# sp-uhh/disentangled-vae

Hardware: AMD Instinct MI355X
Metric: spectrogram frames/sec (train step), M2 VAE 513-bin (higher is better)
Workload: dtype bf16x3; 1 GPU; M2 VAE train step (fwd+ELBO+bwd+Adam), x_dim 513, y_dim 513, z 16, h [128,128], 8192 frames/step/GPU, 16 kHz / 1024-pt STFT power frames; parallelism=dp1, min_hbm_bytes_per_frame=4168

## Files before the change

### disentangled-vae_amd/csrc/rows_common.hpp

```cpp
#pragma once
#include "fused_tiles.hpp"
#include "apply_types.hpp"

namespace dvae {
namespace fused {

__device__ __forceinline__ void philox_normal4(unsigned long long seed, unsigned long long frame, unsigned long long step, unsigned draw,
                                               float (&out)[4]) {
    unsigned c0 = (unsigned)frame, c1 = (unsigned)(frame >> 32), c2 = (unsigned)step, c3 = ((unsigned)(step >> 32) << 8) | draw;
    unsigned k0 = (unsigned)seed, k1 = (unsigned)(seed >> 32);
#pragma unroll
    for (int r = 0; r < 10; ++r) {
        const unsigned h0 = __umulhi(0xD2511F53u, c0), l0 = 0xD2511F53u * c0;
        const unsigned h1 = __umulhi(0xCD9E8D57u, c2), l1 = 0xCD9E8D57u * c2;
        c0 = h1 ^ c1 ^ k0; c1 = l1; c2 = h0 ^ c3 ^ k1; c3 = l0;
        k0 += 0x9E3779B9u; k1 += 0xBB67AE85u;
    }
    const float u0 = ((float)(c0 >> 8) + 0.5f) * (1.f / 16777216.f), u1 = ((float)(c1 >> 8) + 0.5f) * (1.f / 16777216.f);
    const float u2 = ((float)(c2 >> 8) + 0.5f) * (1.f / 16777216.f), u3 = ((float)(c3 >> 8) + 0.5f) * (1.f / 16777216.f);
    const float ra = sqrtf(-2.f * __logf(u0)), rb = sqrtf(-2.f * __logf(u2));
    float sa, ca, sb, cb;
    __sincosf(6.283185307179586f * u1, &sa, &ca);
    __sincosf(6.283185307179586f * u3, &sb, &cb);
    out[0] = ra * ca; out[1] = ra * sa; out[2] = rb * cb; out[3] = rb * sb;
// ... 128 lines not shown
                if (fbase + l31 >= col_limit) f[j] = P::cvt(0.f);
            }
            stash_store16(dbase, (l31 * E + gq * 32 * E) * (int)sizeof(T), f);
        }
    }
}

template <typename P, bool F16 = false, typename RowOf>
__device__ __forceinline__ void load_rows_to_lds(const float* __restrict__ src, int ld, int ncols, int pcols, int64_t b0, int64_t B,
                                                 typename P::T* U, int ldu, int tid, RowOf rowof, float* xf = nullptr,
                                                 float* log2sum = nullptr, float eps = 0.f) {
    const int total = TB * pcols;
    for (int idx = tid; idx < total; idx += 256) {
        const int row = idx / pcols, col = idx - row * pcols;
        float v = 0.f;
        if (col < ncols && b0 + row < B) {
            v = src[rowof(row) * ld + col];
            if (log2sum && col < XD - 1) *log2sum += __builtin_amdgcn_logf(v + eps);
        }
        if constexpr (F16 && P::NP == 2) {
            const float vs = v * X16::XS;
            const typename P::T vh = X16::hi<typename P::T>(vs);
            U[row * ldu + col] = vh;
            U[Pl<P>::lds + row * ldu + col] = X16::hi<typename P::T>(vs - X16::val(vh));
        } else {
            const typename P::T vh = P::cvt(v);
            U[row * ldu + col] = vh;
            if constexpr (P::NP == 2) U[Pl<P>::lds + row * ldu + col] = P::cvt(v - (float)vh);
        }
        if (xf && col < ncols) xf[row * ncols + col] = v;
    }
}

constexpr int NQ513 = 17;
struct __attribute__((packed, aligned(4))) F4U { f32x4 v; };
#ifndef R2_IN_NT
#define R2_IN_NT 0
#endif
typedef f32x4 f32x4_a4 __attribute__((aligned(4)));
__device__ __forceinline__ f32x4 ld_in4(const float* p) {
#if R2_IN_NT >= 1
    return __builtin_nontemporal_load(reinterpret_cast<const f32x4_a4*>(p));
#else
    return reinterpret_cast<const F4U*>(p)->v;
#endif
}
__device__ __forceinline__ f32x4 ld_in4_again(const float* p) {
#if R2_IN_NT >= 2
    return __builtin_nontemporal_load(reinterpret_cast<const f32x4_a4*>(p));
#else
    return reinterpret_cast<const F4U*>(p)->v;
#endif
}
template <int I0, int I1, typename RowOf>
__device__ __forceinline__ void tile513_issue_part(const float* __restrict__ base, RowOf rowof, f32x4 (&v)[NQ513], int tid) {
#pragma unroll
    for (int i = I0; i < I1; ++i) {
        const int c = tid + 256 * i;
        v[i] = ld_in4(base + rowof(c >> 7) * XD + 4 * (c & 127));
    }
}
template <typename RowOf>
__device__ __forceinline__ void tile513_issue_last(const float* __restrict__ base, RowOf rowof, f32x4 (&v)[NQ513], int tid) {
    v[16][0] = base[rowof(tid & 31) * XD + XD - 1];
}
template <typename RowOf>
__device__ __forceinline__ void tile513_issue(const float* __restrict__ base, RowOf rowof, f32x4 (&v)[NQ513], int tid) {
    tile513_issue_part<0, 16>(base, rowof, v, tid);
    tile513_issue_last(base, rowof, v, tid);
    __builtin_amdgcn_sched_barrier(0);
}
template <typename P, int I0, int I1, bool F16 = false>
__device__ __forceinline__ void tile513_commit_part(const f32x4 (&v)[NQ513], typename P::T* U, int ldu, int tid, float* xf, unsigned long long& lo_bits) {
    typedef typename P::Pack4 Pack4;
#pragma unroll
    for (int i = I0; i < I1; ++i) {
        const int c = tid + 256 * i;
        const int row = c >> 7, col = 4 * (c & 127);
        if (xf) {
            float* d = xf + row * XD + col;
            d[0] = v[i][0]; d[1] = v[i][1]; d[2] = v[i][2]; d[3] = v[i][3];
        }
        if constexpr (F16 && P::NP == 2) {
            Pack4 pk, pl;
#pragma unroll
            for (int j = 0; j < 4; ++j) {
                const float vs = v[i][j] * X16::XS;
                pk[j] = X16::hi<typename P::T>(vs);
                pl[j] = X16::hi<typename P::T>(vs - X16::val(pk[j]));
            }
            *reinterpret_cast<Pack4*>(U + row * ldu + col) = pk;
            *reinterpret_cast<Pack4*>(U + Pl<P>::lds + row * ldu + col) = pl;
            continue;
        }
        Pack4 pk;
        pk[0] = P::cvt(v[i][0]); pk[1] = P::cvt(v[i][1]); pk[2] = P::cvt(v[i][2]); pk[3] = P::cvt(v[i][3]);
        *reinterpret_cast<Pack4*>(U + row * ldu + col) = pk;
        if constexpr (P::NP == 2) {
            Pack4 pl;
            pl[0] = P::cvt(v[i][0] - (float)pk[0]); pl[1] = P::cvt(v[i][1] - (float)pk[1]);
            pl[2] = P::cvt(v[i][2] - (float)pk[2]); pl[3] = P::cvt(v[i][3] - (float)pk[3]);
            *reinterpret_cast<Pack4*>(U + Pl<P>::lds + row * ldu + col) = pl;
            lo_bits |= __builtin_bit_cast(unsigned long long, pl) & 0x7fff7fff7fff7fffull;
        }
    }
}
template <typename P, int PCOLS, bool F16 = false>
__device__ __forceinline__ void tile513_commit_last(const f32x4 (&v)[NQ513], typename P::T* U, int ldu, int tid, float* xf, unsigned long long& lo_bits) {
    constexpr int PADC = PCOLS - XD;
    if (tid < TB) {
        if (xf) xf[tid * XD + XD - 1] = v[16][0];
// ... 107 lines not shown
```

### disentangled-vae_amd/csrc/rows_helper.inc

```
        const int hw = wave_u - ROWS_CHAIN_WAVES, ht = tid - 64 * ROWS_CHAIN_WAVES;
        constexpr bool XFH = P::XF16 && NP == 2;
        constexpr int NBT = Ld<T>::nbias;
        constexpr int NB = (NBT + 255) / 256;
        float bvv[NB];
        auto load_bias = [&]() __attribute__((always_inline)) {
#pragma unroll
            for (int q = 0; q < NB; ++q) {
                int i = ht + 256 * q;
                i = i < NBT ? i : NBT - 1;
                const float* src;
                int k;
                if (i < OB2) { src = g.b1; k = i; }
                else if (i < OBMV) { src = g.b2; k = i - OB2; }
                else if (i < OBMV + ZD) { src = g.bmu; k = i - OBMV; }
                else if (i < OB3) { src = g.blv; k = i - OBMV - ZD; }
                else if (i < OB4) { src = g.b3; k = i - OB3; }
                else if (i < OB5) { src = g.b4; k = i - OB4; }
                else if (i < OB5 + NO) { src = g.b5; k = i - OB5; k = k < XD ? k : XD - 1; }
                else { src = g.w5last; k = i - OB5 - NO; }
                if constexpr (DEFER) bvv[q] = __hip_atomic_load(src + k, __ATOMIC_RELAXED, __HIP_MEMORY_SCOPE_AGENT);
                else bvv[q] = src[k];
            }
        };
        auto store_bias = [&]() __attribute__((always_inline)) {
// ... 23 lines not shown
            hws.pl = g.wpl_bytes;
            auto mo = [&](const void* Wp) { return (unsigned)((const char*)Wp - (const char*)g.wcopy); };
            constexpr unsigned FBB = HS::FBB;
            const unsigned tw = (unsigned)hw * FBB;
            hws.sb[H_W1X] = mo(g.W1s) + tw + (unsigned)SCc::NX1 * 4u * FBB;
            hws.sb[H_W3Y] = mo(g.W3s) + tw + (unsigned)(ZD / KS) * 4u * FBB;
            hws.sb[H_W3Z] = mo(g.W3s) + tw;
            hws.sb[H_PAD] = mo(g.W1s);
            if constexpr (INFO) { hws.sb[H_C1] = mo(g.Wc1s) + tw;  hws.sb[H_C2] = mo(g.Wc2s) + tw;  hws.sb[H_C2T] = mo(g.Wc2t) + tw; }
            else { hws.sb[H_C1] = hws.sb[H_C2] = hws.sb[H_C2T] = 0; }
            if constexpr (INFO) hws.fill();
        }
        const T* const Urh = U + l31 * LDU + h * E;
        const T* const Zbrh = Zb + l31 * LDZ + h * E;
        float lsum2 = 0.f;
        f32x4 xv[NQ513], yv[NQ513];
        bool x_in_regs = false;
        bool y_in_regs = false;
        const bool st1 = MODE != 1 && !(g.ablate & 1), st2 = MODE != 1 && !(g.ablate & 2) && (g.stash_inputs & 2), st2x = MODE != 1 && !(g.ablate & 2) && (g.stash_inputs & 1);
        for (int it = 0; it < ntl; ++it) {
            const int tile = tile0 + it * (int)gridDim.x;
            const int64_t b0 = (int64_t)tile * TB;
            const bool full = (b0 + TB) <= g.B;
            const int64_t* const rsrc = rowsrc + (it & 1) * TB;
            auto rowof = [&](int r) -> int64_t {
                if (gather) return rsrc[r];
                const int64_t br = b0 + r;
                return br < g.B ? br : g.B - 1;
            };
            int tl = ht;
            asm volatile("" : "+v"(tl));
            const bool yfast = Y513 && g.fasty && full;
            bool y_early = it > 0 && y_in_regs;
            if (it == 0) {
                if (gather) { fill_rows(tile, 0); wg_barrier(); }
                if (g.fastx && full) {
                    tile513_issue(g.x, rowof, xv, tl);
                    if constexpr (!DEFER) store_bias();
#if R2_EARLY_Y
                    if (YP > 0 && Y513 && g.fasty) {
                        unsigned long long lb = 0ull;
                        static_for<0, 4>([&](auto qc) {
                            constexpr int Q = decltype(qc)::value;
                            tile513_issue_part<4 * Q, 4 * Q + 4>(g.y, rowof, yv, tl);
                            __builtin_amdgcn_sched_barrier(0);
                            tile513_commit_part<P, 4 * Q, 4 * Q + 4, XFH>(xv, U, LDU, tl, nullptr, lb);
                            __builtin_amdgcn_sched_barrier(0);
                        });
                        tile513_issue_last(g.y, rowof, yv, tl);
                        __builtin_amdgcn_sched_barrier(0);
                        tile513_commit_last<P, ROWS_XP, XFH>(xv, U, LDU, tl, nullptr, lb);
                        y_early = true;
                    } else
#endif
                    {
                        tile513_commit<P, ROWS_XP, XFH>(xv, U, LDU, tl);
#pragma unroll
                        for (int i = 0; i < NQ513; ++i) yv[i] = f32x4{0.f, 0.f, 0.f, 0.f};
                    }
                } else {
#pragma unroll
                    for (int i = 0; i < NQ513; ++i) { xv[i] = f32x4{0.f, 0.f, 0.f, 0.f}; yv[i] = f32x4{0.f, 0.f, 0.f, 0.f}; }
                    if constexpr (!DEFER) store_bias();
                    load_rows_to_lds<P, XFH>(g.x, g.ldx, XD, ROWS_XP, b0, g.B, U, LDU, tl, rowof, nullptr, OFFL ? &lsum2 : nullptr, g.elbo_eps);
                }
                if constexpr (INFO) {
                    for (int i = ht; i < 6 * HD + 2; i += 256) {
                        const int q = i / HD, k = i - q * HD;
                        float v;
                        if (q == 0) v = g.bc1[k]; else if (q == 1) v = g.bc2[k]; else if (q == 2) v = g.wc3[k];
                        else if (q == 3) v = g.ba1[k]; else if (q == 4) v = g.ba2[k]; else if (q == 5) v = g.wa3[k];
                        else v = k == 0 ? g.bc3[0] : g.ba3[0];
                        Binfo[i] = v;
                    }
                }
                if (ht == 0) flags[0] = 0;
                if constexpr (DEFER) {
                    wg_barrier();
                    load_bias();
                    store_bias();
                }
                wg_barrier();
                if constexpr (OFFL) { if (g.fastx && full) lsum2 += tile513_log2sum(xv, g.elbo_eps, tl); }
            }
            if constexpr (HS::n(H_W1X) > 0) {
                f32x16 hacc;
                zero_acc<P>(hacc);
                hws.fill();
                gemm_seg<P, HS, DH, H_W1X, HWS, XFH>(hacc, hws, Urh + SCc::NX1 * 2 * E);
#pragma unroll
                for (int r = 0; r < 16; ++r) keep[r * 256 + ht] = XFH ? hacc[r] * X16::ACC : hacc[r];
            }
            float c1r[16], c2r[16], w3c[16];
            float bce_c = 0.f, ylab = 0.f;
            if constexpr (INFO) {
                ylab = g.y[rowof(l31) * g.ldy];
                if (it > 0) hws.fill();
                f32x16 cacc;
                zero_acc<P>(cacc);
                gemm_seg<P, HS, DH, H_C1, HWS, XFH>(cacc, hws, Urh);
                float bvc[16];
                bias16(Binfo + OBC1, 32 * hw, h, bvc);
#pragma unroll
                for (int r = 0; r < 16; ++r) c1r[r] = fmaxf((XFH ? cacc[r] * X16::ACC : cacc[r]) + bvc[r], 0.f);
            }
            f32x16 accy;
            int yplanes = NP;
            int ydirty = 0;
            if constexpr (NP == 2 && YP > 0) { if (g.ylo_skip && st2) ydirty = g.ylo_dirty[tile]; }
            if (YP > 0) {
                if (Y513 && yfast && !y_early) tile513_issue(g.y, rowof, yv, tl);
                R2_HSTAMP(16);
                if (st2x && !XFH) stash_from_lds<P>(U, LDU, ROWS_XP, NO, (T*)g.xT, g.spl, g.Bp, b0, tl);
                R2_HSTAMP(17);
                wg_barrier();
                if constexpr (HS::HELPY && HS::n(H_W1X) == 0) hws.fill();
                R2_HSTAMP(18);
                bool any = false;
                if (Y513 && yfast) tile513_commit<P, ROWS_XP>(yv, U, LDU, tl, nullptr, NP == 2 ? &any : nullptr);
                else load_rows_to_lds<P>(g.y, g.ldy, g.ydim, YP, b0, g.B, U, LDU, tl, rowof);
                R2_HSTAMP(19);
                if constexpr (NP == 2) {
                    if (Y513 && yfast) {
                    } else {
                        constexpr int YPD = YP > 0 ? YP : 1;
                        for (int idx = tl; idx < TB * YP; idx += 256) any |= (float)U[Pl<P>::lds + (idx / YPD) * LDU + idx % YPD] != 0.f;
                    }
                    if (__ballot(any) != 0ull && lane == 0) atomicOr(&flags[0], 1);
                }
                R2_HSTAMP(20);
                if constexpr (INFO) put_lds<P>(c1r, U + IMA, LDU, 32 * hw, l31, h);
                wg_barrier();
                if constexpr (NP == 2) {
                    const bool ylo_t = __builtin_amdgcn_readfirstlane(flags[0]) != 0;
                    if (g.ylo_skip && st2) {
                        ydirty = __builtin_amdgcn_readfirstlane(ydirty);
                        yplanes = (ylo_t || ydirty != 0) ? 2 : 1;
                        if (ht == 0) {
                            if (ylo_t) *g.ylo_epoch = g.launch_id;
                            if ((ylo_t ? 1 : 0) != ydirty) g.ylo_dirty[tile] = ylo_t ? 1 : 0;
                        }
                    }
                }
#if !R2_LATE_Y
                if (st2) stash_from_lds<P>(U, LDU, YP, (YP + 31) / 32 * 32, (T*)g.yT, g.spl, g.Bp, b0, tl, 0, 1 << 30, yplanes);
#endif
                if constexpr (HS::HELPY) {
                    const bool ylo = NP == 2 && __builtin_amdgcn_readfirstlane(flags[0]) != 0;
                    zero_acc<P>(accy);
                    if (!R2_YLOSEG) gemm_seg<P, HS, DH, H_W3Y>(accy, hws, Urh, ylo);
                    else if (ylo) gemm_seg<P, HS, DH, H_W3Y>(accy, hws, Urh, true);
                    else gemm_seg<P, HS, DH, H_W3Y>(accy, hws, Urh, false);
                }
                if constexpr (INFO) {
                    f32x16 a2c;
                    zero_acc<P>(a2c);
                    gemm_seg<P, HS, DH, H_C2>(a2c, hws, Urh + IMA);
                    float bvc[16];
                    bias16(Binfo + OBC2, 32 * hw, h, bvc);
                    bias16(Binfo + OWC3, 32 * hw, h, w3c);
                    float pd = 0.f;
#pragma unroll
                    for (int r = 0; r < 16; ++r) { c2r[r] = fmaxf(a2c[r] + bvc[r], 0.f); pd = fmaf(w3c[r], c2r[r], pd); }
                    put_lds<P>(c2r, U + IMB, LDU, 32 * hw, l31, h);
                    pd += __shfl_xor(pd, 32, 64);
                    if (h == 0) red2[hw * 32 + l31] = pd;
                }
            } else {
                if (st2x && !XFH) stash_from_lds<P>(U, LDU, ROWS_XP, NO, (T*)g.xT, g.spl, g.Bp, b0, tl);
                if constexpr (HS::n(H_W1X) > 0) wg_barrier();
            }
            wg_barrier();
            if constexpr (INFO) {
                const bool live_h = (b0 + l31) < g.B;
                const float logit = red2[l31] + red2[32 + l31] + red2[64 + l31] + red2[96 + l31] + Binfo[OS3];
                const float p = 1.f / (1.f + P::exp_(-logit));
                const float lp = P::log_(p + g.elbo_eps), lq = P::log_(1.f - p + g.elbo_eps);
                bce_c = (live_h && h == 0 && hw == 0) ? -(ylab * lp + (1.f - ylab) * lq) : 0.f;
                const float u = live_h ? -g.invB * (ylab / (p + g.elbo_eps) - (1.f - ylab) / (1.f - p + g.elbo_eps)) : 0.f;
                const float dpre3 = u * p * (1.f - p);
                float dv2[16];
#pragma unroll
                for (int r = 0; r < 16; ++r) dv2[r] = c2r[r] > 0.f ? w3c[r] * dpre3 : 0.f;
                put_lds<P>(dv2, U + IMC, LDU, 32 * hw, l31, h);
                if (st1) {
// ... 208 lines not shown
```

### disentangled-vae_amd/csrc/rows_prologue.inc

```
    typedef typename P::T T;
    typedef typename P::Frag Frag;
    constexpr int E = P::E, KS = P::KSTEP, NP = P::NP;
    constexpr int LDU = Ld<T>::u, LDH = Ld<T>::hh, LDZ = Ld<T>::z;
    constexpr bool Y513 = (YP == ROWS_XP);
#ifndef R2_OFFL
#define R2_OFFL 1
#endif
#ifndef R2_LATE_Y
#define R2_LATE_Y 1
#endif
#ifndef R2_EARLY_Y
#define R2_EARLY_Y 1
#endif
#ifndef R2_DH
#define R2_DH 6
#endif
#ifndef R2_HPRIO
#define R2_HPRIO 0
#endif
#ifndef R2_YSPREAD
#define R2_YSPREAD 8
#endif
#ifndef R2_YLOSEG
#define R2_YLOSEG 0
#endif
#ifndef R2_STAGGER
#define R2_STAGGER 0
#endif
    constexpr bool OFFL = R2_OFFL && MODE == 0 && NP == 2;
    extern __shared__ __attribute__((aligned(16))) char smem[];
    T* const U = reinterpret_cast<T*>(smem);
    T* const Ha = U + TB * LDU;
    T* const Hb = Ha + TB * LDH;
    T* const Zb = Hb + TB * LDH;
    typedef Lds2<P, INFO> LD2;
    float* const Bias = reinterpret_cast<float*>(smem + LD2::o_bias);
    float* const red = reinterpret_cast<float*>(smem + LD2::o_red);
    int* const flags = reinterpret_cast<int*>(smem + LD2::o_flags);
    int64_t* const rowsrc = reinterpret_cast<int64_t*>(smem + LD2::o_rows);
    float* const Binfo = reinterpret_cast<float*>(smem + LD2::o_info);
    float* const red2 = reinterpret_cast<float*>(smem + LD2::o_red2);
    float* const dzs = reinterpret_cast<float*>(smem + LD2::o_dzu);
    constexpr int OBC1 = 0, OBC2 = HD, OWC3 = 2 * HD, OBA1 = 3 * HD, OBA2 = 4 * HD, OWA3 = 5 * HD, OS3 = 6 * HD;
    constexpr int IMA = 32, IMB = 160, IMC = 288;
    float* const keep = reinterpret_cast<float*>(smem + LD2::o_keep);
    float* const keepz = reinterpret_cast<float*>(smem + LD2::o_keepz);
    constexpr int OB1 = 0, OB2 = HD, OBMV = 2 * HD, OB3 = 2 * HD + 32, OB4 = 3 * HD + 32, OB5 = 4 * HD + 32;

    constexpr int DH = R2_DH;
    const int tid = threadIdx.x, lane = tid & 63;
    const int wave_u = __builtin_amdgcn_readfirstlane(tid >> 6);
    const int l31 = lane & 31, h = lane >> 5;
    const bool gather = g.rows != nullptr;
#ifndef R2_XCDMAP
#define R2_XCDMAP 0
#endif
    int tile0 = (int)blockIdx.x;
#if R2_XCDMAP
    if ((gridDim.x & 7) == 0 && (g.ntiles % (int)gridDim.x) == 0) tile0 = (int)(blockIdx.x & 7) * (int)(gridDim.x >> 3) + (int)(blockIdx.x >> 3);
#endif
    const int ntl = (g.ntiles - tile0 + (int)gridDim.x - 1) / (int)gridDim.x;

// ... 1 lines not shown
```

### disentangled-vae_amd/csrc/train_rows2.hip

```cpp
#include <math.h>
#include <stdlib.h>
#include "fused_tiles.hpp"
#include "rows_common.hpp"
#include "wstream.hpp"
#include "apply_common.hpp"
#include "rows_shared.hpp"
#include "../../include/dvae_train.h"

namespace dvae {
namespace fused {

template <typename P, int YP, bool YENC, int MODE, bool INFO = false, bool DEFER = false>
__global__ __launch_bounds__(512) void vae_rows2_kernel(const RowsArgs g) {
    static_assert(!INFO || (MODE == 0 && YP == 16 && !YENC), "M2_info: train step, 1-dim label, encoder on x only");
    static_assert(!DEFER || (MODE == 0 && !INFO && sizeof(typename P::T) == 2), "deferred optimizer step: M1 / M2 train step, bf16 copies");
#define ROWS_XP XP
#define ROWS_PREFETCH 1
#define ROWS_CHAIN_WAVES 4
#include "rows_prologue.inc"
    if (wave_u < 4) {
        const int cw = wave_u, fb = 32 * cw;
        constexpr int D = OFFL ? P::PDO : P::PD;
        typedef Sched<P, YP, YENC, D, INFO> SC;
        typedef HSched<P, YP, YENC, DH, INFO> HS;
#ifndef R2_DEFER_WAUX
#define R2_DEFER_WAUX 0
#endif
        typedef WStream<P, SC, D, DEFER ? R2_DEFER_WAUX : R2_WAUX> WS;
        constexpr unsigned FBB = SC::FBB;
        WS ws;
        ws.rs = __builtin_amdgcn_make_buffer_rsrc(const_cast<void*>(g.wcopy), 0, (int)g.wcopy_bytes, 0x00020000);
        ws.voff = lane * 16;
        ws.pl = g.wpl_bytes;
        {
            auto mo = [&](const void* Wp) { return (unsigned)((const char*)Wp - (const char*)g.wcopy); };
#ifdef R2_SAMEW
            const unsigned tw = 0;
#else
            const unsigned tw = (unsigned)cw * FBB;
#endif
            constexpr unsigned KB1 = (XP / KS) * 4 * FBB, KB3 = (ZD / KS) * 4 * FBB;
            ws.sb[G_W1X] = mo(g.W1s) + tw;  ws.sb[G_W1Y] = mo(g.W1s) + tw + KB1;
            ws.sb[G_W2] = mo(g.W2s) + tw;   ws.sb[G_WMV] = mo(g.Wmvs);
            ws.sb[G_W3Y] = mo(g.W3s) + tw + KB3;  ws.sb[G_W3Z] = mo(g.W3s) + tw;
            ws.sb[G_W4] = mo(g.W4s) + tw;
            ws.sb[G_W5A] = mo(g.W5s) + (unsigned)cw * FBB;        ws.sb[G_W5B] = mo(g.W5s) + (unsigned)(cw + 4) * FBB;
            ws.sb[G_W5C] = mo(g.W5s) + (unsigned)(cw + 8) * FBB;  ws.sb[G_W5D] = mo(g.W5s) + (unsigned)(cw + 12) * FBB;
            ws.sb[G_W5T] = mo(g.W5t) + tw;  ws.sb[G_W4T] = mo(g.W4t) + tw;  ws.sb[G_W3ZT] = mo(g.W3zt);
            ws.sb[G_WMVT] = mo(g.Wmvt) + tw;  ws.sb[G_W2T] = mo(g.W2t) + tw;  ws.sb[G_PAD] = mo(g.W1s);
            if constexpr (INFO) {
// ... 26 lines not shown
            wg_barrier();
        }
        ws.fill();
        const T* const Ur = U + l31 * LDU + h * E;
        const T* const Har = Ha + l31 * LDH + h * E;
        const T* const Hbr = Hb + l31 * LDH + h * E;
        const T* const Zbr = Zb + l31 * LDZ + h * E;
        const bool w0 = cw == 0;
        constexpr int mode = MODE;
        double tot_rec = 0.0, tot_kl = 0.0, tot_bc = 0.0, tot_ba = 0.0;

        for (int it = 0; it < ntl; ++it) {
            const int tile = tile0 + it * (int)gridDim.x;
            const int64_t b0 = (int64_t)tile * TB;
            const bool live = (b0 + l31) < g.B;
            const int64_t* const rsrc = rowsrc + (it & 1) * TB;
            float rec_lane = 0.f, kl_lane = 0.f;
            R2_STAMP(0);
            if (g.dbg && tid == 0) g.dbg[(size_t)blockIdx.x * 32 + 30] = clock64();
            float ep_r[8];
            if (w0) {
                int64_t br = b0 + l31; br = br < g.B ? br : g.B - 1;
                if (g.eps != nullptr) {
                    const f32x4 e0 = *reinterpret_cast<const f32x4*>(g.eps + br * ZD + 4 * h);
                    const f32x4 e1 = *reinterpret_cast<const f32x4*>(g.eps + br * ZD + 8 + 4 * h);
#pragma unroll
                    for (int jq = 0; jq < 4; ++jq) { ep_r[jq] = live ? e0[jq] : 0.f; ep_r[4 + jq] = live ? e1[jq] : 0.f; }
                } else {
                    frame_noise8(g.rng_seed, (unsigned long long)br, g.rng_step, h, ep_r);
#pragma unroll
                    for (int jq = 0; jq < 8; ++jq) ep_r[jq] = live ? ep_r[jq] : 0.f;
                }
            }
            if (it == 0) {
                if (gather) wg_barrier();
                wg_barrier();
            }
            R2_STAMP(1);
#if R2_STAGGER
            if (it == 0) { for (int q = 0; q < (int)((blockIdx.x >> 3) & 7); ++q) __builtin_amdgcn_s_sleep(R2_STAGGER); }
#endif
            f32x16 acc;
            zero_acc<P>(acc);
            constexpr bool XF = P::XF16 && NP == 2;
            gemm_seg<P, SC, D, G_W1X, WS, XF>(acc, ws, Ur);
            if constexpr (XF) {
#pragma unroll
                for (int r = 0; r < 16; ++r) acc[r] *= X16::ACC;
            }
            R2_STAMP(2);
            bool ylo = false;
            if (YP > 0) {
                wg_barrier();
                wg_barrier();
                ylo = NP == 2 && __builtin_amdgcn_readfirstlane(flags[0]) != 0;
                if (!R2_YLOSEG) gemm_seg<P, SC, D, G_W1Y>(acc, ws, Ur, ylo);
                else if (ylo) gemm_seg<P, SC, D, G_W1Y>(acc, ws, Ur, true);
                else gemm_seg<P, SC, D, G_W1Y>(acc, ws, Ur, false);
            } else if constexpr (HS::n(H_W1X) > 0) wg_barrier();
            if constexpr (HS::n(H_W1X) > 0) {
#pragma unroll
                for (int r = 0; r < 16; ++r) acc[r] += keep[r * 256 + tid];
            }
            float hv[16], bv[16];
            R2_STAMP(3);
            bias16(Bias + OB1, fb, h, bv);
#pragma unroll
            for (int r = 0; r < 16; ++r) { hv[r] = P::tanh_(acc[r] + bv[r]); keep[r * 256 + tid] = hv[r]; }
            put_lds<P>(hv, Ha, LDH, fb, l31, h);
            wg_barrier();
            R2_STAMP(4);
            zero_acc<P>(acc);
            gemm_seg<P, SC, D, G_W2>(acc, ws, Har);
            bias16(Bias + OB2, fb, h, bv);
#pragma unroll
            for (int r = 0; r < 16; ++r) { hv[r] = P::tanh_(acc[r] + bv[r]); keep[(16 + r) * 256 + tid] = hv[r]; }
            put_lds<P>(hv, Hb, LDH, fb, l31, h);
            wg_barrier();
            R2_STAMP(5);
            zero_acc<P>(acc);
            gemm_seg<P, SC, D, G_WMV>(acc, ws, Hbr, true, w0);
            if (w0) {
                float zv[16];
                bias16(Bias + OBMV, 0, h, bv);
#pragma unroll
                for (int r = 0; r < 8; ++r) {
                    const float mu = acc[r] + bv[r], lv = acc[r + 8] + bv[r + 8];
                    keepz[r * 64 + lane] = mu; keepz[(8 + r) * 64 + lane] = lv;
                    zv[r] = fmaf(P::exp_(0.5f * lv), ep_r[r], mu);
                    zv[r + 8] = 0.f;
                    if (live) kl_lane += lv - mu * mu - P::exp_(lv);
                }
                put_lds<P>(zv, Zb, LDZ, 0, l31, h);
                if (mode == 1 && live) {
                    const int64_t o = (b0 + l31) * ZD + 4 * h;
#pragma unroll
                    for (int q = 0; q < 2; ++q) {
                        *reinterpret_cast<f32x4*>(g.out_mu + o + 8 * q) = f32x4{acc[4 * q] + bv[4 * q], acc[4 * q + 1] + bv[4 * q + 1], acc[4 * q + 2] + bv[4 * q + 2], acc[4 * q + 3] + bv[4 * q + 3]};
                        *reinterpret_cast<f32x4*>(g.out_lv + o + 8 * q) = f32x4{acc[8 + 4 * q] + bv[8 + 4 * q], acc[9 + 4 * q] + bv[9 + 4 * q], acc[10 + 4 * q] + bv[10 + 4 * q], acc[11 + 4 * q] + bv[11 + 4 * q]};
                        if (g.out_z) *reinterpret_cast<f32x4*>(g.out_z + o + 8 * q) = f32x4{zv[4 * q], zv[4 * q + 1], zv[4 * q + 2], zv[4 * q + 3]};
                    }
                }
            }
            f32x16 accy;
            if constexpr (YP > 0 && !SC::HELPY) {
                zero_acc<P>(accy);
                if (!R2_YLOSEG) gemm_seg<P, SC, D, G_W3Y>(accy, ws, Ur, ylo);
                else if (ylo) gemm_seg<P, SC, D, G_W3Y>(accy, ws, Ur, true);
                else gemm_seg<P, SC, D, G_W3Y>(accy, ws, Ur, false);
            }
            wg_barrier();
            R2_STAMP(6);
            float bce_a = 0.f;
            if constexpr (INFO) {
                float a1r[16], a2r[16], w3v[16];
                zero_acc<P>(acc);
                gemm_seg<P, SC, D, G_A1>(acc, ws, Zbr);
                bias16(Binfo + OBA1, fb, h, bv);
#pragma unroll
                for (int r = 0; r < 16; ++r) a1r[r] = fmaxf(acc[r] + bv[r], 0.f);
                put_lds<P>(a1r, Ha, LDH, fb, l31, h);
                wg_barrier();
                zero_acc<P>(acc);
                gemm_seg<P, SC, D, G_A2>(acc, ws, Har);
                bias16(Binfo + OBA2, fb, h, bv);
                bias16(Binfo + OWA3, fb, h, w3v);
                float pd = 0.f;
#pragma unroll
                for (int r = 0; r < 16; ++r) { a2r[r] = fmaxf(acc[r] + bv[r], 0.f); pd = fmaf(w3v[r], a2r[r], pd); }
                put_lds<P>(a2r, Hb, LDH, fb, l31, h);
                pd += __shfl_xor(pd, 32, 64);
                if (h == 0) red2[cw * 32 + l31] = pd;
                wg_barrier();
                {
                    int64_t rowy = gather ? rsrc[l31] : (b0 + l31 < g.B ? b0 + l31 : g.B - 1);
                    const float y_l = g.y[rowy * g.ldy];
                    const float logit = red2[l31] + red2[32 + l31] + red2[64 + l31] + red2[96 + l31] + Binfo[OS3 + 1];
                    const float p = 1.f / (1.f + P::exp_(-logit));
                    const float lp = P::log_(p + g.elbo_eps), lq = P::log_(1.f - p + g.elbo_eps);
                    bce_a = (live && h == 0 && w0) ? -(y_l * lp + (1.f - y_l) * lq) : 0.f;
                    const float u = live ? -g.invB * (y_l / (p + g.elbo_eps) - (1.f - y_l) / (1.f - p + g.elbo_eps)) : 0.f;
                    const float dpre3 = u * p * (1.f - p);
// ... 219 lines not shown
            for (int r = 0; r < 16; ++r) { const float hk = keep[r * 256 + tid]; dv[r] = acc[r] * (1.f - hk * hk); }
            put_lds<P>(dv, Ha, LDH, fb, l31, h);
            wg_barrier();
            R2_STAMP(14);
            if (!live) rec_lane = 0.f;
            const float rs = wave_sum(rec_lane), ks = wave_sum(kl_lane);
            if (lane == 0) { red[cw] = rs; red[4 + cw] = ks; }
            if constexpr (INFO) { if (w0) { const float bas = wave_sum(bce_a); if (lane == 0) red2[129] = bas; } }
            wg_barrier();
            if (tid == 0) {
                if constexpr (INFO) { tot_bc += (double)red2[128]; tot_ba += (double)red2[129]; }
                tot_rec += (double)red[0] + (double)red[1] + (double)red[2] + (double)red[3];
                if constexpr (OFFL)
                    tot_rec += (double)red[8] + (double)red[9] + (double)red[10] + (double)red[11]
                             - 0.6931471805599453 * ((double)red[12] + (double)red[13] + (double)red[14] + (double)red[15]);
                tot_kl += -0.5 * (double)red[4];
            }
        }
        R2_STAMP(15);
        if (g.dbg && tid == 0) g.dbg[(size_t)blockIdx.x * 32 + 31] = clock64();
        if (tid == 0) {
            g.partials[4 * blockIdx.x] = tot_rec;
            g.partials[4 * blockIdx.x + 1] = tot_kl;
            g.partials[4 * blockIdx.x + 2] = tot_bc;
            g.partials[4 * blockIdx.x + 3] = tot_ba;
        }
    } else {
#include "rows_helper.inc"
    }
}

#undef ROWS_XP
#undef ROWS_CHAIN_WAVES
template <typename P, int YP, bool YENC, int MODE, bool INFO = false, bool DEFER = false>
static int launch_rows2_m(const RowsArgs& a, int grid, hipStream_t s) {
    const size_t lds = Lds2<P, INFO>::bytes;
    static bool attr_done[64] = {};
    int dev = 0;
    (void)hipGetDevice(&dev);
    if (dev < 0 || dev >= 64) dev = 0;
    if (!attr_done[dev]) {
        hipError_t e = hipFuncSetAttribute((const void*)vae_rows2_kernel<P, YP, YENC, MODE, INFO, DEFER>, hipFuncAttributeMaxDynamicSharedMemorySize, (int)lds);
        if (e != hipSuccess) { set_error("hipFuncSetAttribute(rows2 kernel, %zu B LDS): %s", lds, hipGetErrorString(e)); return (int)e; }
        attr_done[dev] = true;
    }
    hipLaunchKernelGGL((vae_rows2_kernel<P, YP, YENC, MODE, INFO, DEFER>), dim3(grid), dim3(512), lds, s, a);
    DVAE_LAUNCH_OK("vae_rows2_kernel");
    return 0;
}

template <typename P, int YP, bool YENC>
static int launch_rows2_t(const RowsArgs& a, int grid, hipStream_t s) {
    if (a.mode == 1) return launch_rows2_m<P, YP, YENC, 1>(a, grid, s);
    if (a.mode == 2) return launch_rows2_m<P, YP, YENC, 2>(a, grid, s);
#ifdef DVAE_DIAG
    if (a.defer.on) return launch_rows2_m<P, YP, YENC, 0, false, true>(a, grid, s);
#else
    if (a.defer.on) { set_error("rows2 kernel: the deferred optimizer step exists in the diagnostic build only (build.py --diag)"); return DVAE_E_UNSUPPORTED; }
#endif
    return launch_rows2_m<P, YP, YENC, 0>(a, grid, s);
}

int launch_rows2(int precision, int model, int y_dim, const RowsArgs& a, int grid, hipStream_t s) {
    const bool m2 = model == DVAE_MODEL_M2;
    if (model == DVAE_MODEL_M2_INFO) {
        if (a.mode != 0) { set_error("rows2 kernel: M2_info runs the fused train step only (mode %d)", a.mode); return DVAE_E_UNSUPPORTED; }
// ... 29 lines not shown
```

### disentangled-vae_amd/csrc/wstream.hpp

```cpp
#pragma once
#include <type_traits>
#include "fused_tiles.hpp"

#ifndef R2_WAUX
#define R2_WAUX 0
#endif
#ifndef R2_NX1
#define R2_NX1 33
#endif
#ifndef R2_HELPY
#define R2_HELPY 0
#endif

namespace dvae {
namespace fused {

enum { G_W1X, G_W1Y, G_W2, G_WMV, G_W3Y, G_A1, G_A2, G_A2T, G_A1T, G_W3Z, G_W4, G_W5A, G_W5B, G_W5C, G_W5D, G_W5T, G_W4T, G_W3ZT, G_WMVT, G_W2T, G_PAD, G_N };

template <typename P, int YP, bool YENC, int D, bool INFO = false> struct Sched {
    static constexpr int KS = P::KSTEP;
    static constexpr int NSEG = G_N;
    static constexpr unsigned FBB = 64u * P::E * sizeof(typename P::T);
    static constexpr int NX1 = (R2_NX1 > 0 && R2_NX1 < XP / KS) ? R2_NX1 : XP / KS;
    static constexpr bool HELPY = R2_HELPY && YP == XP;
// ... 44 lines not shown
    __amdgpu_buffer_rsrc_t rs;
    int voff;
    unsigned pl;
    unsigned sb[SC::NSEG];
    unsigned cur;
    template <int Q> __device__ __forceinline__ void req() {
        constexpr int s = SC::seg_of(Q);
        if constexpr (Q == SC::start(s)) cur = sb[s];
        else cur += SC::stride(s);
        asm volatile("" : "+s"(cur));
        const u32x4 v0 = __builtin_amdgcn_raw_buffer_load_b128(rs, voff, cur, AUX);
        r[Q % D][0] = __builtin_bit_cast(typename P::Frag, v0);
        if constexpr (P::NP == 2) {
            const u32x4 v1 = __builtin_amdgcn_raw_buffer_load_b128(rs, voff, cur + pl, AUX);
            r[Q % D][1] = __builtin_bit_cast(typename P::Frag, v1);
        }
    }
    template <int S, int SLOT> __device__ __forceinline__ void req_next() {
        cur += SC::stride(S);
        asm volatile("" : "+s"(cur));
        const u32x4 v0 = __builtin_amdgcn_raw_buffer_load_b128(rs, voff, cur, AUX);
        r[SLOT][0] = __builtin_bit_cast(typename P::Frag, v0);
        if constexpr (P::NP == 2) {
            const u32x4 v1 = __builtin_amdgcn_raw_buffer_load_b128(rs, voff, cur + pl, AUX);
            r[SLOT][1] = __builtin_bit_cast(typename P::Frag, v1);
        }
    }
    __device__ __forceinline__ void fill() {
        static_for<0, (D < SC::total ? D : SC::total)>([&](auto ic) { this->template req<decltype(ic)::value>(); });
        __builtin_amdgcn_sched_barrier(0);
    }
};

template <typename P, typename SC, int D, int S, typename WS, bool F16 = false>
__device__ __forceinline__ void gemm_seg(f32x16& acc, WS& w, const typename P::T* brow, bool blo = true, bool active = true) {
    typedef typename P::Frag Frag;
    constexpr int N = SC::n(S), Q0 = SC::start(S), STR = 2 * P::E;
    if constexpr (N > 0) {
        constexpr int BD = N < P::BDMAX ? N : P::BDMAX;
        Frag bq[BD][P::NP];
        if (active) {
#pragma unroll
            for (int i = 0; i < BD; ++i) bloadp<P>(bq[i], brow + i * STR);
        }
#ifndef R2_ROLL
#define R2_ROLL 0
#endif
        constexpr int NL = (R2_ROLL && D % BD == 0 && N >= 3 * D) ? (N - D) / D : 0;
        constexpr int NR = NL * D;
        if constexpr (NL > 0) {
            const typename P::T* bl = brow;
#pragma unroll 1
            for (int lap = 0; lap < NL; ++lap) {
                static_for<0, D>([&](auto ic) {
                    constexpr int i = decltype(ic)::value;
                    if (active) {
#ifndef R2_NOMFMA
                        if constexpr (F16) mmap_f16<P>(acc, w.r[(Q0 + i) % D], bq[i % BD]);
                        else mmap<P>(acc, w.r[(Q0 + i) % D], bq[i % BD], blo);
#else
                        acc[0] += (float)w.r[(Q0 + i) % D][0][0] + (float)bq[i % BD][0][0];
#endif
#ifndef R2_NOBLOAD
                        bloadp<P>(bq[i % BD], bl + (i + BD) * STR);
#endif
                    }
#ifndef R2_NOWLOAD
                    w.template req_next<S, (Q0 + i) % D>();
#endif
                    __builtin_amdgcn_sched_barrier(0);
                });
                bl += D * STR;
            }
        }
        static_for<NR, N>([&](auto ic) {
            constexpr int I = decltype(ic)::value;
            if (active) {
#ifndef R2_NOMFMA
                if constexpr (F16) mmap_f16<P>(acc, w.r[(Q0 + I) % D], bq[I % BD]);
                else mmap<P>(acc, w.r[(Q0 + I) % D], bq[I % BD], blo);
#else
                acc[0] += (float)w.r[(Q0 + I) % D][0][0] + (float)bq[I % BD][0][0];
#endif
#ifndef R2_NOBLOAD
                if constexpr (I + BD < N) bloadp<P>(bq[I % BD], brow + (I + BD) * STR);
#endif
            }
#ifndef R2_NOWLOAD
            if constexpr (SC::WRAP) w.template req<(Q0 + I + D) % SC::total>();
            else if constexpr (Q0 + I + D < SC::total) w.template req<Q0 + I + D>();
#endif
            __builtin_amdgcn_sched_barrier(0);
        });
    }
}

}
}
```

Baseline: 108.8 million frames/s.

## Split input tiles into column bands with per-band label lo-plane skipping

Adds an optional streamed opening that loads and commits the x and y tiles in four column bands, with a barrier per band. This lets the first-layer GEMM start on early bands while later bands are still arriving. It also replaces the single label 'low plane nonzero' flag with one flag per band group, so the y GEMMs can skip the bf16x3 low-plane MFMAs band by band. The streamed opening and its band-major tile map are off by default behind macros. The per-band flagging and split label GEMM do run by default, and they add extra B-fragment prefetch restarts at group boundaries plus extra ballots.

After: 108.8 million frames/s (median of 6 runs). No clear change (-0.0%).

```diff
diff --git a/disentangled-vae_amd/csrc/rows_common.hpp b/disentangled-vae_amd/csrc/rows_common.hpp
--- a/disentangled-vae_amd/csrc/rows_common.hpp
+++ b/disentangled-vae_amd/csrc/rows_common.hpp
@@ -184,7 +184,21 @@
     }
 }
 
+#ifndef R2_XSTREAM
+#define R2_XSTREAM 0
+#endif
+#ifndef R2_BANDMAP
+#define R2_BANDMAP (R2_XSTREAM ? 1 : 2)
+#endif
 constexpr int NQ513 = 17;
+constexpr int NBG = 4;
+__device__ __forceinline__ constexpr int band_group(int col) { return col >> 7 < NBG - 1 ? col >> 7 : NBG - 1; }
+__device__ __forceinline__ int tile513_row(int i, int tid) {
+    return R2_BANDMAP == 2 ? (tid + 256 * i) >> 7 : R2_BANDMAP == 1 ? 8 * (i & 3) + (tid >> 5) : tid >> 3;
+}
+__device__ __forceinline__ int tile513_col(int i, int tid) {
+    return R2_BANDMAP == 2 ? 4 * ((tid + 256 * i) & 127) : R2_BANDMAP == 1 ? 128 * (i >> 2) + 4 * (tid & 31) : 32 * i + 4 * (tid & 7);
+}
 struct __attribute__((packed, aligned(4))) F4U { f32x4 v; };
 #ifndef R2_IN_NT
 #define R2_IN_NT 0
@@ -208,8 +222,7 @@
 __device__ __forceinline__ void tile513_issue_part(const float* __restrict__ base, RowOf rowof, f32x4 (&v)[NQ513], int tid) {
 #pragma unroll
     for (int i = I0; i < I1; ++i) {
-        const int c = tid + 256 * i;
-        v[i] = ld_in4(base + rowof(c >> 7) * XD + 4 * (c & 127));
+        v[i] = ld_in4(base + rowof(tile513_row(i, tid)) * XD + tile513_col(i, tid));
     }
 }
 template <typename RowOf>
@@ -227,8 +240,7 @@
     typedef typename P::Pack4 Pack4;
 #pragma unroll
     for (int i = I0; i < I1; ++i) {
-        const int c = tid + 256 * i;
-        const int row = c >> 7, col = 4 * (c & 127);
+        const int row = tile513_row(i, tid), col = tile513_col(i, tid);
         if (xf) {
             float* d = xf + row * XD + col;
             d[0] = v[i][0]; d[1] = v[i][1]; d[2] = v[i][2]; d[3] = v[i][3];
diff --git a/disentangled-vae_amd/csrc/rows_helper.inc b/disentangled-vae_amd/csrc/rows_helper.inc
--- a/disentangled-vae_amd/csrc/rows_helper.inc
+++ b/disentangled-vae_amd/csrc/rows_helper.inc
@@ -79,11 +79,37 @@
             asm volatile("" : "+v"(tl));
             const bool yfast = Y513 && g.fasty && full;
             bool y_early = it > 0 && y_in_regs;
+            const bool xstream = XSTREAM && it == 0 && g.fastx && g.fasty && full;
             if (it == 0) {
                 if (gather) { fill_rows(tile, 0); wg_barrier(); }
                 if (g.fastx && full) {
                     tile513_issue(g.x, rowof, xv, tl);
                     if constexpr (!DEFER) store_bias();
+                    if (xstream) {
+                        if (ht == 0) flags[0] = 0;
+                        unsigned long long lb = 0ull;
+                        static_for<0, NBG>([&](auto qc) {
+                            constexpr int Q = decltype(qc)::value;
+                            tile513_issue_part<4 * Q, 4 * Q + 4>(g.y, rowof, yv, tl);
+                            if constexpr (Q == NBG - 1) tile513_issue_last(g.y, rowof, yv, tl);
+                            __builtin_amdgcn_sched_barrier(0);
+                            tile513_commit_part<P, 4 * Q, 4 * Q + 4, XFH>(xv, U, LDU, tl, nullptr, lb);
+                            if constexpr (Q == NBG - 1) tile513_commit_last<P, ROWS_XP, XFH>(xv, U, LDU, tl, nullptr, lb);
+                            R2_HSTAMP(16 + Q);
+                            wg_barrier();
+                        });
+                        if constexpr (OFFL) lsum2 += tile513_log2sum(xv, g.elbo_eps, tl);
+                        static_for<0, NBG>([&](auto qc) {
+                            constexpr int Q = decltype(qc)::value;
+                            unsigned long long yb = 0ull;
+                            tile513_commit_part<P, 4 * Q, 4 * Q + 4>(yv, U, LDU, tl, nullptr, yb);
+                            if constexpr (Q == NBG - 1) tile513_commit_last<P, ROWS_XP>(yv, U, LDU, tl, nullptr, yb);
+                            if constexpr (NP == 2) { if (__ballot(yb != 0ull) != 0ull && lane == 0) atomicOr(&flags[0], 1 << Q); }
+                            if constexpr (Q == NBG - 1) R2_HSTAMP(20);
+                            wg_barrier();
+                        });
+                        y_early = true;
+                    } else
 #if R2_EARLY_Y
                     if (YP > 0 && Y513 && g.fasty) {
                         unsigned long long lb = 0ull;
@@ -121,14 +147,16 @@
                         Binfo[i] = v;
                     }
                 }
-                if (ht == 0) flags[0] = 0;
-                if constexpr (DEFER) {
+                if (!xstream) {
+                    if (ht == 0) flags[0] = 0;
+                    if constexpr (DEFER) {
+                        wg_barrier();
+                        load_bias();
+                        store_bias();
+                    }
                     wg_barrier();
-                    load_bias();
-                    store_bias();
-                }
-                wg_barrier();
-                if constexpr (OFFL) { if (g.fastx && full) lsum2 += tile513_log2sum(xv, g.elbo_eps, tl); }
+                    if constexpr (OFFL) { if (g.fastx && full) lsum2 += tile513_log2sum(xv, g.elbo_eps, tl); }
+                }
             }
             if constexpr (HS::n(H_W1X) > 0) {
                 f32x16 hacc;
@@ -156,6 +184,7 @@
             int ydirty = 0;
             if constexpr (NP == 2 && YP > 0) { if (g.ylo_skip && st2) ydirty = g.ylo_dirty[tile]; }
             if (YP > 0) {
+              if (!xstream) {
                 if (Y513 && yfast && !y_early) tile513_issue(g.y, rowof, yv, tl);
                 R2_HSTAMP(16);
                 if (st2x && !XFH) stash_from_lds<P>(U, LDU, ROWS_XP, NO, (T*)g.xT, g.spl, g.Bp, b0, tl);
@@ -163,21 +192,33 @@
                 wg_barrier();
                 if constexpr (HS::HELPY && HS::n(H_W1X) == 0) hws.fill();
                 R2_HSTAMP(18);
-                bool any = false;
-                if (Y513 && yfast) tile513_commit<P, ROWS_XP>(yv, U, LDU, tl, nullptr, NP == 2 ? &any : nullptr);
-                else load_rows_to_lds<P>(g.y, g.ldy, g.ydim, YP, b0, g.B, U, LDU, tl, rowof);
+                unsigned long long yb[NBG] = {0ull, 0ull, 0ull, 0ull};
+                if (Y513 && yfast) {
+                    static_for<0, NBG>([&](auto qc) {
+                        constexpr int Q = decltype(qc)::value;
+                        tile513_commit_part<P, 4 * Q, 4 * Q + 4>(yv, U, LDU, tl, nullptr, yb[Q]);
+                    });
+                    tile513_commit_last<P, ROWS_XP>(yv, U, LDU, tl, nullptr, yb[NBG - 1]);
+                } else load_rows_to_lds<P>(g.y, g.ldy, g.ydim, YP, b0, g.B, U, LDU, tl, rowof);
                 R2_HSTAMP(19);
                 if constexpr (NP == 2) {
                     if (Y513 && yfast) {
                     } else {
                         constexpr int YPD = YP > 0 ? YP : 1;
-                        for (int idx = tl; idx < TB * YP; idx += 256) any |= (float)U[Pl<P>::lds + (idx / YPD) * LDU + idx % YPD] != 0.f;
-                    }
-                    if (__ballot(any) != 0ull && lane == 0) atomicOr(&flags[0], 1);
+                        for (int idx = tl; idx < TB * YP; idx += 256) {
+                            const int col = idx % YPD;
+                            if ((float)U[Pl<P>::lds + (idx / YPD) * LDU + col] != 0.f) yb[Y513 ? band_group(col) : 0] = 1ull;
+                        }
+                    }
+                    int bits = 0;
+#pragma unroll
+                    for (int q = 0; q < NBG; ++q) bits |= __ballot(yb[q] != 0ull) != 0ull ? 1 << q : 0;
+                    if (bits != 0 && lane == 0) atomicOr(&flags[0], bits);
                 }
                 R2_HSTAMP(20);
                 if constexpr (INFO) put_lds<P>(c1r, U + IMA, LDU, 32 * hw, l31, h);
                 wg_barrier();
+              }
                 if constexpr (NP == 2) {
                     const bool ylo_t = __builtin_amdgcn_readfirstlane(flags[0]) != 0;
                     if (g.ylo_skip && st2) {
@@ -193,11 +234,9 @@
                 if (st2) stash_from_lds<P>(U, LDU, YP, (YP + 31) / 32 * 32, (T*)g.yT, g.spl, g.Bp, b0, tl, 0, 1 << 30, yplanes);
 #endif
                 if constexpr (HS::HELPY) {
-                    const bool ylo = NP == 2 && __builtin_amdgcn_readfirstlane(flags[0]) != 0;
+                    const int yfl = NP == 2 ? __builtin_amdgcn_readfirstlane(flags[0]) : 0;
                     zero_acc<P>(accy);
-                    if (!R2_YLOSEG) gemm_seg<P, HS, DH, H_W3Y>(accy, hws, Urh, ylo);
-                    else if (ylo) gemm_seg<P, HS, DH, H_W3Y>(accy, hws, Urh, true);
-                    else gemm_seg<P, HS, DH, H_W3Y>(accy, hws, Urh, false);
+                    label_gemm<P, HS, DH, H_W3Y, Y513>(accy, hws, Urh, [&](int) { return yfl; });
                 }
                 if constexpr (INFO) {
                     f32x16 a2c;
diff --git a/disentangled-vae_amd/csrc/rows_prologue.inc b/disentangled-vae_amd/csrc/rows_prologue.inc
--- a/disentangled-vae_amd/csrc/rows_prologue.inc
+++ b/disentangled-vae_amd/csrc/rows_prologue.inc
@@ -28,6 +28,12 @@
 #define R2_STAGGER 0
 #endif
     constexpr bool OFFL = R2_OFFL && MODE == 0 && NP == 2;
+#ifndef ROWS_XSTREAM
+#define ROWS_XSTREAM 0
+#endif
+    constexpr bool XSTREAM = ROWS_XSTREAM && R2_EARLY_Y && MODE == 0 && Y513 && YENC && !INFO && !DEFER && P::XF16 && NP == 2 &&
+                             Sched<P, YP, YENC, 1, INFO>::NX1 == XP / KS && !Sched<P, YP, YENC, 1, INFO>::HELPY;
+    static_assert(!XSTREAM || R2_BANDMAP != 2, "the streamed opening needs a band-major tile map (rows_common.hpp: R2_BANDMAP 0 / 1)");
     extern __shared__ __attribute__((aligned(16))) char smem[];
     T* const U = reinterpret_cast<T*>(smem);
     T* const Ha = U + TB * LDU;
diff --git a/disentangled-vae_amd/csrc/train_rows2.hip b/disentangled-vae_amd/csrc/train_rows2.hip
--- a/disentangled-vae_amd/csrc/train_rows2.hip
+++ b/disentangled-vae_amd/csrc/train_rows2.hip
@@ -16,6 +16,7 @@
     static_assert(!DEFER || (MODE == 0 && !INFO && sizeof(typename P::T) == 2), "deferred optimizer step: M1 / M2 train step, bf16 copies");
 #define ROWS_XP XP
 #define ROWS_PREFETCH 1
+#define ROWS_XSTREAM R2_XSTREAM
 #define ROWS_CHAIN_WAVES 4
 #include "rows_prologue.inc"
     if (wave_u < 4) {
@@ -108,6 +109,7 @@
                     for (int jq = 0; jq < 8; ++jq) ep_r[jq] = live ? ep_r[jq] : 0.f;
                 }
             }
+            const bool xstream = XSTREAM && it == 0 && g.fastx && g.fasty && b0 + TB <= g.B;
             if (it == 0) {
                 if (gather) wg_barrier();
                 wg_barrier();
@@ -119,20 +121,28 @@
             f32x16 acc;
             zero_acc<P>(acc);
             constexpr bool XF = P::XF16 && NP == 2;
-            gemm_seg<P, SC, D, G_W1X, WS, XF>(acc, ws, Ur);
+            if constexpr (XSTREAM) {
+                static_for<0, 4>([&](auto qc) {
+                    constexpr int Q = decltype(qc)::value;
+                    if constexpr (Q > 0) { if (xstream) wg_barrier(); }
+                    gemm_group<P, SC, D, G_W1X, WS, XF, Q>(acc, ws, Ur);
+                });
+            } else gemm_seg<P, SC, D, G_W1X, WS, XF>(acc, ws, Ur);
             if constexpr (XF) {
 #pragma unroll
                 for (int r = 0; r < 16; ++r) acc[r] *= X16::ACC;
             }
             R2_STAMP(2);
-            bool ylo = false;
+            int yfl = 0;
             if (YP > 0) {
-                wg_barrier();
-                wg_barrier();
-                ylo = NP == 2 && __builtin_amdgcn_readfirstlane(flags[0]) != 0;
-                if (!R2_YLOSEG) gemm_seg<P, SC, D, G_W1Y>(acc, ws, Ur, ylo);
-                else if (ylo) gemm_seg<P, SC, D, G_W1Y>(acc, ws, Ur, true);
-                else gemm_seg<P, SC, D, G_W1Y>(acc, ws, Ur, false);
+                if (!xstream) {
+                    wg_barrier();
+                    wg_barrier();
+                }
+                label_gemm<P, SC, D, G_W1Y, Y513>(acc, ws, Ur, [&](int q) {
+                    if (xstream) wg_barrier();
+                    return yfl = NP == 2 ? __builtin_amdgcn_readfirstlane(flags[0]) : 0;
+                });
             } else if constexpr (HS::n(H_W1X) > 0) wg_barrier();
             if constexpr (HS::n(H_W1X) > 0) {
 #pragma unroll
@@ -181,9 +191,7 @@
             f32x16 accy;
             if constexpr (YP > 0 && !SC::HELPY) {
                 zero_acc<P>(accy);
-                if (!R2_YLOSEG) gemm_seg<P, SC, D, G_W3Y>(accy, ws, Ur, ylo);
-                else if (ylo) gemm_seg<P, SC, D, G_W3Y>(accy, ws, Ur, true);
-                else gemm_seg<P, SC, D, G_W3Y>(accy, ws, Ur, false);
+                label_gemm<P, SC, D, G_W3Y, Y513>(accy, ws, Ur, [&](int) { return yfl; });
             }
             wg_barrier();
             R2_STAMP(6);
@@ -469,6 +477,7 @@
 
 #undef ROWS_XP
 #undef ROWS_CHAIN_WAVES
+#undef ROWS_XSTREAM
 template <typename P, int YP, bool YENC, int MODE, bool INFO = false, bool DEFER = false>
 static int launch_rows2_m(const RowsArgs& a, int grid, hipStream_t s) {
     const size_t lds = Lds2<P, INFO>::bytes;
diff --git a/disentangled-vae_amd/csrc/wstream.hpp b/disentangled-vae_amd/csrc/wstream.hpp
--- a/disentangled-vae_amd/csrc/wstream.hpp
+++ b/disentangled-vae_amd/csrc/wstream.hpp
@@ -100,22 +100,24 @@
     }
 };
 
-template <typename P, typename SC, int D, int S, typename WS, bool F16 = false>
+template <typename P, typename SC, int D, int S, typename WS, bool F16 = false, int K0 = 0, int K1 = -1>
 __device__ __forceinline__ void gemm_seg(f32x16& acc, WS& w, const typename P::T* brow, bool blo = true, bool active = true) {
     typedef typename P::Frag Frag;
-    constexpr int N = SC::n(S), Q0 = SC::start(S), STR = 2 * P::E;
-    if constexpr (N > 0) {
-        constexpr int BD = N < P::BDMAX ? N : P::BDMAX;
+    constexpr int NS = SC::n(S), Q0 = SC::start(S), STR = 2 * P::E;
+    constexpr int N = K1 < 0 || K1 > NS ? NS : K1;
+    static_assert(K0 >= 0 && (K0 == 0 || K0 < N), "k-step range");
+    if constexpr (N > K0) {
+        constexpr int BD = N - K0 < P::BDMAX ? N - K0 : P::BDMAX;
         Frag bq[BD][P::NP];
         if (active) {
 #pragma unroll
-            for (int i = 0; i < BD; ++i) bloadp<P>(bq[i], brow + i * STR);
+            for (int i = K0; i < K0 + BD; ++i) bloadp<P>(bq[i % BD], brow + i * STR);
         }
 #ifndef R2_ROLL
 #define R2_ROLL 0
 #endif
-        constexpr int NL = (R2_ROLL && D % BD == 0 && N >= 3 * D) ? (N - D) / D : 0;
-        constexpr int NR = NL * D;
+        constexpr int NL = (R2_ROLL && K0 == 0 && N == NS && D % BD == 0 && N >= 3 * D) ? (N - D) / D : 0;
+        constexpr int NR = NL > 0 ? NL * D : K0;
         if constexpr (NL > 0) {
             const typename P::T* bl = brow;
 #pragma unroll 1
@@ -163,5 +165,36 @@
     }
 }
 
-}
-}
+template <typename P, typename SC, int D, int S, typename WS, bool F16, int Q>
+__device__ __forceinline__ void gemm_group(f32x16& acc, WS& w, const typename P::T* brow, bool blo = true) {
+    static_assert(SC::n(S) == 33 && P::KSTEP == 16, "band groups: 33 k-steps of 16");
+    gemm_seg<P, SC, D, S, WS, F16, 8 * Q, Q == 3 ? -1 : 8 * Q + 8>(acc, w, brow, blo);
+}
+#ifndef R2_YLOSEG
+#define R2_YLOSEG 0
+#endif
+template <typename P, typename SC, int D, int S, bool GROUPS, typename WS, typename FlagOf>
+__device__ __forceinline__ void label_gemm(f32x16& acc, WS& w, const typename P::T* brow, FlagOf&& flag_of) {
+    auto run = [&](auto qc, bool lo) __attribute__((always_inline)) {
+        constexpr int Q = decltype(qc)::value;
+        if constexpr (Q < 0) {
+            if (!R2_YLOSEG) gemm_seg<P, SC, D, S, WS>(acc, w, brow, lo);
+            else if (lo) gemm_seg<P, SC, D, S, WS>(acc, w, brow, true);
+            else gemm_seg<P, SC, D, S, WS>(acc, w, brow, false);
+        } else {
+            if (!R2_YLOSEG) gemm_group<P, SC, D, S, WS, false, Q>(acc, w, brow, lo);
+            else if (lo) gemm_group<P, SC, D, S, WS, false, Q>(acc, w, brow, true);
+            else gemm_group<P, SC, D, S, WS, false, Q>(acc, w, brow, false);
+        }
+    };
+    if constexpr (GROUPS) {
+        static_for<0, 4>([&](auto qc) {
+            constexpr int Q = decltype(qc)::value;
+            const int f = flag_of(Q);
+            run(qc, P::NP == 2 && ((f >> Q) & 1) != 0);
+        });
+    } else run(std::integral_constant<int, -1>{}, P::NP == 2 && flag_of(0) != 0);
+}
+
+}
+}
```
